# NVlabs/FoundationPose

Hardware: NVIDIA H100
Metric: pose-hypotheses/sec at 640x480 RGB-D, 252 hyp, 5 refine iters (higher is better)
Workload: dtype f16

## Files before the change

foundationpose_b200/csrc/fp_common.cuh:

```cuda
#pragma once
#include <cuda.h>
#include <cuda_fp16.h>
#include <cuda_runtime.h>
#include <stdint.h>
#include <stdio.h>
#include <string.h>

#include <atomic>

namespace fp {

void note_launches(int n);
unsigned long long launch_count();
void set_capturing(bool on);
inline bool device_bit_test(const std::atomic<unsigned long long>& m) {
  int d = 0;
  cudaGetDevice(&d);
  return (m.load(std::memory_order_acquire) >> (d & 63)) & 1ull;
}
inline void device_bit_set(std::atomic<unsigned long long>& m) {
  int d = 0;
  cudaGetDevice(&d);
  m.fetch_or(1ull << (d & 63), std::memory_order_release);
}
int num_sms();

void set_last_error(const char* fmt, ...);
int check_device_ptr(const void* p, const char* what, const char* fn = "fp_pose_errors");
#define FP_CUDA_OK(expr)                                                                   \
  do {                                                                                     \
    cudaError_t _e = (expr);                                                               \
    if (_e != cudaSuccess) {                                                               \
      fp::set_last_error("%s:%d: %s -> %s", __FILE__, __LINE__, #expr, cudaGetErrorString(_e)); \
      return -2;                                                                           \
    }                                                                                      \
  } while (0)
#define FP_REQUIRE(cond, ...)                                                              \
  do {                                                                                     \
    if (!(cond)) {                                                                         \
      fp::set_last_error(__VA_ARGS__);                                                     \
      return -1;                                                                           \
    }                                                                                      \
  } while (0)
#define FP_TRY(expr)     \
  do {                   \
    int _rc = (expr);    \
    if (_rc) return _rc; \
  } while (0)

bool pdl_enabled();
void pdl_skip_next();

template <typename... KArgs, typename... Args>
inline cudaError_t launch_pdl(void (*kernel)(KArgs...), dim3 grid, dim3 block, size_t smem, cudaStream_t stream,
                              int cluster_x, Args... args) {
  cudaLaunchConfig_t cfg;
  memset(&cfg, 0, sizeof(cfg));
  cfg.gridDim = grid;
  cfg.blockDim = block;
  cfg.dynamicSmemBytes = smem;
  cfg.stream = stream;
  cudaLaunchAttribute attr[2];
  int na = 0;
  if (cluster_x > 1) {
    attr[na].id = cudaLaunchAttributeClusterDimension;
    attr[na].val.clusterDim.x = cluster_x;
    attr[na].val.clusterDim.y = 1;
    attr[na].val.clusterDim.z = 1;
    ++na;
  }
  if (pdl_enabled()) {
    attr[na].id = cudaLaunchAttributeProgrammaticStreamSerialization;
    attr[na].val.programmaticStreamSerializationAllowed = 1;
    ++na;
  }
  cfg.attrs = attr;
  cfg.numAttrs = na;
  return cudaLaunchKernelEx(&cfg, kernel, KArgs(args)...);
}

__device__ __forceinline__ void pdl_wait() { asm volatile("griddepcontrol.wait;" ::: "memory"); }
__device__ __forceinline__ void pdl_trigger() { asm volatile("griddepcontrol.launch_dependents;" ::: "memory"); }

__device__ __forceinline__ uint32_t smem_u32(const void* p) {
  return static_cast<uint32_t>(__cvta_generic_to_shared(p));
}

__device__ __forceinline__ void mbar_init(uint64_t* bar, uint32_t count) {
  asm volatile("mbarrier.init.shared::cta.b64 [%0], %1;" ::"r"(smem_u32(bar)), "r"(count));
}
__device__ __forceinline__ void mbar_fence_init() {
  asm volatile("fence.mbarrier_init.release.cluster;" ::: "memory");
}
__device__ __forceinline__ void mbar_expect_tx(uint64_t* bar, uint32_t bytes) {
  asm volatile("mbarrier.arrive.expect_tx.shared::cta.b64 _, [%0], %1;" ::"r"(smem_u32(bar)),
               "r"(bytes)
               : "memory");
}
__device__ __forceinline__ void mbar_arrive(uint64_t* bar) {
  asm volatile("mbarrier.arrive.shared::cta.b64 _, [%0];" ::"r"(smem_u32(bar)) : "memory");
}
__device__ __forceinline__ void mbar_wait(uint64_t* bar, uint32_t parity) {
  asm volatile(
      "{\n\t"
      ".reg .pred P1;\n\t"
      "WAIT_%=:\n\t"
      "mbarrier.try_wait.parity.shared::cta.b64 P1, [%0], %1, %2;\n\t"
      "@P1 bra DONE_%=;\n\t"
      "bra WAIT_%=;\n\t"
      "DONE_%=:\n\t"
      "}" ::"r"(smem_u32(bar)),
      "r"(parity), "r"(0x989680)
      : "memory");
}

__device__ __forceinline__ void tma_load_5d(const CUtensorMap* map, uint64_t* bar, void* dst,
                                            int c0, int c1, int c2, int c3, int c4) {
  asm volatile(
      "cp.async.bulk.tensor.5d.shared::cluster.global.mbarrier::complete_tx::bytes"
      " [%0], [%1, {%3, %4, %5, %6, %7}], [%2];" ::"r"(smem_u32(dst)),
      "l"(reinterpret_cast<uint64_t>(map)), "r"(smem_u32(bar)), "r"(c0), "r"(c1), "r"(c2),
      "r"(c3), "r"(c4)
      : "memory");
}
__device__ __forceinline__ void tma_load_2d(const CUtensorMap* map, uint64_t* bar, void* dst,
                                            int c0, int c1) {
  asm volatile(
      "cp.async.bulk.tensor.2d.shared::cluster.global.mbarrier::complete_tx::bytes"
      " [%0], [%1, {%3, %4}], [%2];" ::"r"(smem_u32(dst)),
      "l"(reinterpret_cast<uint64_t>(map)), "r"(smem_u32(bar)), "r"(c0), "r"(c1)
      : "memory");
}
__device__ __forceinline__ void tma_store_5d(const CUtensorMap* map, const void* src, int c0, int c1, int c2, int c3,
                                             int c4) {
  asm volatile("cp.async.bulk.tensor.5d.global.shared::cta.bulk_group [%0, {%2, %3, %4, %5, %6}], [%1];" ::"l"(
                   reinterpret_cast<uint64_t>(map)),
               "r"(smem_u32(src)), "r"(c0), "r"(c1), "r"(c2), "r"(c3), "r"(c4)
               : "memory");
}
__device__ __forceinline__ void tma_prefetch_desc(const CUtensorMap* map) {
  asm volatile("prefetch.tensormap [%0];" ::"l"(reinterpret_cast<uint64_t>(map)) : "memory");
}

__device__ __forceinline__ uint32_t cluster_nctarank() {
  uint32_t r;
  asm volatile("mov.u32 %0, %%cluster_nctarank;" : "=r"(r));
  return r;
}
__device__ __forceinline__ uint32_t cluster_ctarank() {
  uint32_t r;
  asm volatile("mov.u32 %0, %%cluster_ctarank;" : "=r"(r));
  return r;
}
__device__ __forceinline__ void cluster_sync_all() {
  asm volatile("barrier.cluster.arrive.release.aligned;" ::: "memory");
  asm volatile("barrier.cluster.wait.acquire.aligned;" ::: "memory");
}

template <uint32_t N>
__device__ __forceinline__ void regs_release() {
  asm volatile("setmaxnreg.dec.sync.aligned.u32 %0;" ::"n"(N));
}
template <uint32_t N>
__device__ __forceinline__ void regs_acquire() {
  asm volatile("setmaxnreg.inc.sync.aligned.u32 %0;" ::"n"(N));
}

__device__ __forceinline__ void wgmma_fence() { asm volatile("wgmma.fence.sync.aligned;" ::: "memory"); }
__device__ __forceinline__ void wgmma_commit() { asm volatile("wgmma.commit_group.sync.aligned;" ::: "memory"); }
template <int N>
__device__ __forceinline__ void wgmma_wait() {
  asm volatile("wgmma.wait_group.sync.aligned %0;" ::"n"(N) : "memory");
}
template <int N>
__device__ __forceinline__ void fence_regs(float (&d)[N]) {
#pragma unroll
  for (int i = 0; i < N; ++i) asm volatile("" : "+f"(d[i])::"memory");
}

__device__ __forceinline__ uint64_t gmma_desc_sw128(uint32_t smem_addr, uint32_t sbo = 1024) {
  uint64_t d = 0;
  d |= (uint64_t)((smem_addr & 0x3FFFF) >> 4);
  d |= (uint64_t)1 << 16;
  d |= (uint64_t)(sbo >> 4) << 32;
  d |= (uint64_t)1 << 62;
  return d;
}
__device__ __forceinline__ uint64_t gmma_desc_mn_sw128(uint32_t smem_addr, uint32_t lbo) {
  uint64_t d = 0;
  d |= (uint64_t)((smem_addr & 0x3FFFF) >> 4);
  d |= (uint64_t)((lbo >> 4) & 0x3FFF) << 16;
  d |= (uint64_t)(1024 >> 4) << 32;
  d |= (uint64_t)1 << 62;
  return d;
}
__device__ __forceinline__ uint64_t gmma_desc_linear(uint32_t smem_addr, uint32_t lbo, uint32_t sbo) {
  uint64_t d = 0;
  d |= (uint64_t)((smem_addr & 0x3FFFF) >> 4);
  d |= (uint64_t)(lbo >> 4) << 16;
  d |= (uint64_t)(sbo >> 4) << 32;
  return d;
}

__device__ __forceinline__ void ldsm_x4_trans(uint32_t addr, uint32_t (&r)[4]) {
  asm volatile("ldmatrix.sync.aligned.m8n8.x4.trans.shared.b16 {%0, %1, %2, %3}, [%4];"
               : "=r"(r[0]), "=r"(r[1]), "=r"(r[2]), "=r"(r[3])
               : "r"(addr)
               : "memory");
}
__device__ __forceinline__ void stsm_x4_trans(uint32_t addr, const uint32_t (&r)[4]) {
  asm volatile("stmatrix.sync.aligned.m8n8.x4.trans.shared.b16 [%0], {%1, %2, %3, %4};" ::"r"(addr), "r"(r[0]),
               "r"(r[1]), "r"(r[2]), "r"(r[3])
               : "memory");
}

__device__ __forceinline__ uint32_t pack_half2(float a, float b) {
  __half2 h = __floats2half2_rn(a, b);
  return *reinterpret_cast<uint32_t*>(&h);
}

}
```

foundationpose_b200/csrc/fp_linear.cu:

```cuda
#include <stdlib.h>
#include <string.h>

#include "fp_common.cuh"
#include "fp_gemm.cuh"
#include "fp_wgmma.cuh"

namespace fp {

int encode_map_f16(CUtensorMap* map, const void* base, int rank, const uint64_t* dims, const uint64_t* strides_bytes,
                   const uint32_t* box);

constexpr int kLwsK = 512;
constexpr int kLwsKBlocks = kLwsK / 64;
constexpr int kLwsRows = 64;
constexpr int kLwsCols = 128;
constexpr int kLwsThreads = 384;
constexpr int kLwsBoxBytes = kLwsCols * 64 * 2;
constexpr int kLwsPanelBytes = kLwsKBlocks * kLwsBoxBytes;
constexpr int kLwsStages = kLwsKBlocks;
constexpr int kLwsStageBytes = kLwsRows * 64 * 2;
constexpr int kLwsSlabBytes = kLwsRows * 64 * 2;
constexpr int kLwsSlabs = 4;
constexpr int kLwsSmemBytes =
    kLwsPanelBytes + kLwsStages * kLwsStageBytes + kLwsSlabs * kLwsSlabBytes + 1024  + 256 ;
static_assert(kLwsSmemBytes <= 232448, "the weight-stationary linear kernel exceeds the 227 KB opt-in shared memory");
static_assert((2 * kLwsStages + 4) * 8 <= 256, "the mbarriers must fit their 256 bytes");

constexpr uint32_t kOrderBar = 2;
constexpr uint32_t kWgBar = 4;

struct LinearWsParams {
  int row_tiles;
  int total;
  const float* bias;
  int has_res;
  int relu;
};

__device__ __forceinline__ void named_sync(uint32_t id, uint32_t count) {
  asm volatile("bar.sync %0, %1;" ::"r"(id), "r"(count) : "memory");
}
__device__ __forceinline__ void named_arrive(uint32_t id, uint32_t count) {
  asm volatile("bar.arrive %0, %1;" ::"r"(id), "r"(count) : "memory");
}

__global__ void __launch_bounds__(kLwsThreads, 1)
    linear_ws_kernel(const __grid_constant__ CUtensorMap map_a, const __grid_constant__ CUtensorMap map_w,
                     const __grid_constant__ CUtensorMap map_out, const __grid_constant__ CUtensorMap map_res,
                     const __grid_constant__ LinearWsParams p) {
  extern __shared__ uint8_t smem_raw[];
  uint8_t* smem = smem_raw + ((1024u - (smem_u32(smem_raw) & 1023u)) & 1023u);
  uint8_t* panel = smem;
  uint8_t* ring = panel + kLwsPanelBytes;
  uint8_t* staging = ring + kLwsStages * kLwsStageBytes;
  uint64_t* bars = reinterpret_cast<uint64_t*>(staging + kLwsSlabs * kLwsSlabBytes);
  uint64_t* full = bars;
  uint64_t* empty = bars + kLwsStages;
  uint64_t* panel_full = bars + 2 * kLwsStages;
  uint64_t* panel_empty = panel_full + 1;
  uint64_t* res_full = panel_full + 2;

  const int i0 = (int)((long long)blockIdx.x * p.total / gridDim.x);
  const int n = (int)((long long)(blockIdx.x + 1) * p.total / gridDim.x) - i0;
  const int panel0 = i0 / p.row_tiles;
  const int jb = min(n, (panel0 + 1) * p.row_tiles - i0);
  const bool reload = jb < n;

  if (threadIdx.x == 0) {
    tma_prefetch_desc(&map_a);
    tma_prefetch_desc(&map_w);
    tma_prefetch_desc(&map_out);
    if (p.has_res) tma_prefetch_desc(&map_res);
    for (int s = 0; s < kLwsStages; ++s) {
      mbar_init(&full[s], 1);
      mbar_init(&empty[s], 128);
    }
    mbar_init(panel_full, 1);
    mbar_init(panel_empty, 256);
    mbar_init(&res_full[0], 1);
    mbar_init(&res_full[1], 1);
    mbar_fence_init();
    mbar_expect_tx(panel_full, kLwsPanelBytes);
    for (int kb = 0; kb < kLwsKBlocks; ++kb)
      tma_load_2d(&map_w, panel_full, panel + kb * kLwsBoxBytes, kb * 64, panel0 * kLwsCols);
  }
  __syncthreads();
  pdl_trigger();
  pdl_wait();

  if (threadIdx.x < 128) {
    if (threadIdx.x == 0) {
      for (int j = 0; j < n; ++j) {
        if (j == jb) {
          mbar_wait(panel_empty, 0);
          mbar_expect_tx(panel_full, kLwsPanelBytes);
          for (int kb = 0; kb < kLwsKBlocks; ++kb)
            tma_load_2d(&map_w, panel_full, panel + kb * kLwsBoxBytes, kb * 64, (panel0 + 1) * kLwsCols);
        }
        const int row0 = ((i0 + j) % p.row_tiles) * kLwsRows;
        for (int kb = 0; kb < kLwsKBlocks; ++kb) {
          mbar_wait(&empty[kb], (uint32_t)((j & 1) ^ 1));
          mbar_expect_tx(&full[kb], kLwsStageBytes);
          tma_load_2d(&map_a, &full[kb], ring + kb * kLwsStageBytes, kb * 64, row0);
        }
      }
    }
    return;
  }

  const int ct = threadIdx.x - 128;
  const int w = ct >> 7;
  const int lane = threadIdx.x & 31;
  const int r0 = 16 * ((ct >> 5) & 3) + (lane >> 2);
  const int cq = 2 * (lane & 3);
  const bool leader = (ct & 127) == 0;
  uint8_t* slabs = staging + w * 2 * kLwsSlabBytes;
  if (reload && w >= jb) mbar_arrive(panel_empty);
  float acc[64];
#pragma unroll
  for (int i = 0; i < 64; ++i) acc[i] = 0.f;
  for (int j = w, it = 0; j < n; j += 2, ++it) {
    const int item = i0 + j;
    const int pn = item / p.row_tiles;
    const int row0 = (item - pn * p.row_tiles) * kLwsRows;
    if (j > 0) named_sync(kOrderBar + w, 256);
    mbar_wait(panel_full, j >= jb ? 1u : 0u);
    for (int kb = 0; kb < kLwsKBlocks; ++kb) {
      mbar_wait(&full[kb], (uint32_t)(j & 1));
      const uint64_t da = gmma_desc_sw128(smem_u32(ring + kb * kLwsStageBytes));
      const uint64_t db = gmma_desc_sw128(smem_u32(panel + kb * kLwsBoxBytes));
      wgmma_fence();
#pragma unroll
      for (int k = 0; k < 4; ++k)
        Wgmma<128>::ss(acc, da + (uint64_t)(2 * k), db + (uint64_t)(2 * k), (kb > 0 || k > 0) ? 1u : 0u);
      wgmma_commit();
      if (kb == 0 && leader) {
        asm volatile("cp.async.bulk.wait_group.read 0;" ::: "memory");
        if (p.has_res) {
          mbar_expect_tx(&res_full[w], 2 * kLwsSlabBytes);
          for (int s = 0; s < 2; ++s)
            tma_load_5d(&map_res, &res_full[w], slabs + s * kLwsSlabBytes, pn * kLwsCols + 64 * s, row0, 0, 0, 0);
        }
      }
      if (kb > 0) {
        wgmma_wait<1>();
        mbar_arrive(&empty[kb - 1]);
      }
    }
    if (j + 1 < n) named_arrive(kOrderBar + (w ^ 1), 256);
    wgmma_wait<0>();
    fence_regs(acc);
    mbar_arrive(&empty[kLwsKBlocks - 1]);
    if (reload && j < jb && j + 2 >= jb) mbar_arrive(panel_empty);

    const float* bias = p.bias + pn * kLwsCols;
    if (p.has_res) mbar_wait(&res_full[w], (uint32_t)(it & 1));
    else named_sync(kWgBar + w, 128);
#pragma unroll
    for (int b = 0; b < 2; ++b) {
      uint8_t* slab = slabs + b * kLwsSlabBytes;
#pragma unroll
      for (int jh = 0; jh < 8; jh += 4) {
        float2 bb[4];
        __half2 rv[4][2];
#pragma unroll
        for (int jl = 0; jl < 4; ++jl) {
          bb[jl] = __ldg(reinterpret_cast<const float2*>(bias + 64 * b + 8 * (jh + jl) + cq));
          if (p.has_res) {
#pragma unroll
            for (int h = 0; h < 2; ++h) {
              const int row = r0 + 8 * h;
              rv[jl][h] = *reinterpret_cast<const __half2*>(slab + row * 128 + (((uint32_t)(jh + jl) ^ (uint32_t)(row & 7)) << 4) + cq * 2);
            }
          }
        }
#pragma unroll
        for (int jl = 0; jl < 4; ++jl) {
          const int jc = 8 * b + jh + jl;
#pragma unroll
          for (int h = 0; h < 2; ++h) {
            const int row = r0 + 8 * h;
            uint32_t* cell = reinterpret_cast<uint32_t*>(slab + row * 128 + (((uint32_t)(jh + jl) ^ (uint32_t)(row & 7)) << 4) + cq * 2);
            float a0 = acc[4 * jc + 2 * h] + bb[jl].x, a1 = acc[4 * jc + 2 * h + 1] + bb[jl].y;
            if (p.has_res) {
              const float2 r = __half22float2(rv[jl][h]);
              a0 += r.x;
              a1 += r.y;
            }
            if (p.relu) {
              a0 = fmaxf(a0, 0.f);
              a1 = fmaxf(a1, 0.f);
            }
            *cell = pack_half2(a0, a1);
          }
        }
      }
    }
    asm volatile("fence.proxy.async.shared::cta;" ::: "memory");
    named_sync(kWgBar + w, 128);
    if (leader) {
      for (int s = 0; s < 2; ++s)
        tma_store_5d(&map_out, slabs + s * kLwsSlabBytes, pn * kLwsCols + 64 * s, row0, 0, 0, 0);
      asm volatile("cp.async.bulk.commit_group;" ::: "memory");
    }
  }
  if (leader) asm volatile("cp.async.bulk.wait_group 0;" ::: "memory");
}

static bool linear_ws_enabled() {
  const char* e = getenv("FPOSE_LINEAR_WS");
  return !(e && e[0] == '0');
}

constexpr int kLinearWsMinItemsPerCta = 8;

bool linear_ws_takes(const GemmLayer& L) {
  if (L.kind != LK_LINEAR || L.Cin != kLwsK || L.Cout % kLwsCols != 0 || L.out_split != 0 || L.post_add ||
      !linear_ws_enabled())
    return false;
  const int sms = num_sms();
  const int panels = L.Cout / kLwsCols;
  const long long items = (long long)panels * ((L.Win + kLwsRows - 1) / kLwsRows);
  return sms > 0 && panels <= sms && items >= (long long)kLinearWsMinItemsPerCta * sms;
}

int linear_ws_launch(const GemmLayer& L, cudaStream_t stream) {
  const uint64_t E = 2;
  const int M = L.Win;
  LinearWsParams p;
  memset(&p, 0, sizeof(p));
  p.row_tiles = (M + kLwsRows - 1) / kLwsRows;
  p.total = (L.Cout / kLwsCols) * p.row_tiles;
  p.bias = L.bias;
  p.has_res = L.res != nullptr;
  p.relu = L.relu;
  CUtensorMap ma, mw, mo, mr;
  {
    const uint64_t d[2] = {(uint64_t)kLwsK, (uint64_t)M}, s[1] = {(uint64_t)kLwsK * E};
    const uint32_t b[2] = {64, kLwsRows};
    if (int rc = encode_map_f16(&ma, L.in, 2, d, s, b)) return rc;
  }
  {
    const uint64_t d[2] = {(uint64_t)kLwsK, (uint64_t)L.Cout}, s[1] = {(uint64_t)kLwsK * E};
    const uint32_t b[2] = {64, kLwsCols};
    if (int rc = encode_map_f16(&mw, L.w, 2, d, s, b)) return rc;
  }
  auto rows_map = [&](CUtensorMap* m, const void* base, int ld) {
    const uint64_t row = (uint64_t)ld * E;
    const uint64_t d[5] = {(uint64_t)ld, (uint64_t)M, 1, 1, 1}, s[4] = {row, row * M, row * M, row * M};
    const uint32_t b[5] = {64, kLwsRows, 1, 1, 1};
    return encode_map_f16(m, base, 5, d, s, b);
  };
  if (int rc = rows_map(&mo, L.out, L.out_ld)) return rc;
  mr = mo;
  if (L.res) {
    if (int rc = rows_map(&mr, L.res, L.res_ld)) return rc;
  }

  static std::atomic<unsigned long long> attr_mask{0};
  if (!device_bit_test(attr_mask)) {
    FP_CUDA_OK(cudaFuncSetAttribute(linear_ws_kernel, cudaFuncAttributeMaxDynamicSharedMemorySize, kLwsSmemBytes));
    device_bit_set(attr_mask);
  }
  const int sms = num_sms();
  FP_REQUIRE(sms > 0, "no CUDA device");
  const int grid = p.total < sms ? p.total : sms;
  prof_mark_begin(0, 2.0 * (double)M * L.Cout * kLwsK, stream);
  FP_CUDA_OK(launch_pdl(linear_ws_kernel, dim3(grid), dim3(kLwsThreads), kLwsSmemBytes, stream, 1, ma, mw, mo, mr, p));
  prof_mark_end(stream);
  note_launches(1);
  FP_CUDA_OK(cudaGetLastError());
  return 0;
}

}
```

foundationpose_b200/csrc/fp_stem.cu:

```cuda
#include <stdlib.h>
#include <string.h>

#include "fp_common.cuh"
#include "fp_gemm.cuh"
#include "fp_wgmma.cuh"

namespace fp {

int encode_map_f16(CUtensorMap* map, const void* base, int rank, const uint64_t* dims, const uint64_t* strides_bytes,
                   const uint32_t* box);
int encode_map_f16_linear(CUtensorMap* map, const void* base, int rank, const uint64_t* dims,
                          const uint64_t* strides_bytes, const uint32_t* box);
int num_sms();

namespace {

constexpr int kThreadsStem = 384;
constexpr int kTileH = 16, kTileW = 8;
constexpr int kPatchRows = 2 * (kTileH - 1) + 7;
constexpr int kPatchPairs = kTileW + 3;
constexpr int kParStride = kPatchPairs * 16;
constexpr int kRowStride = 2 * kParStride;
constexpr int kPatchBytes = kPatchRows * kRowStride;
constexpr int kPatchSlot = 13 * 1024;
constexpr int kStagesStem = 6;
constexpr int kWTileBytes = 2 * 64 * 16;
constexpr int kWBytes = 28 * kWTileBytes;
constexpr int kHalfSlab = 64 * 64 * 2;
constexpr int kStemSmem = kWBytes + kStagesStem * kPatchSlot + 4 * kHalfSlab + 1024 + 256;

struct StemParams {
  int tiles_w, tiles_h, n_img, total_tiles;
  const float* bias;
  int relu;
};

__device__ __forceinline__ void bulk_load_1d(void* dst, const void* src, uint32_t bytes, uint64_t* bar) {
  asm volatile("cp.async.bulk.shared::cluster.global.mbarrier::complete_tx::bytes [%0], [%1], %2, [%3];" ::"r"(
                   smem_u32(dst)),
               "l"(src), "r"(bytes), "r"(smem_u32(bar))
               : "memory");
}

__global__ void __launch_bounds__(kThreadsStem, 1)
    stem_conv_kernel(const __grid_constant__ CUtensorMap map_in, const __grid_constant__ CUtensorMap map_out,
                     const __half* __restrict__ wpack, const StemParams p) {
  constexpr int S = kStagesStem;
  extern __shared__ uint8_t smem_raw[];
  uint8_t* smem = reinterpret_cast<uint8_t*>((reinterpret_cast<uintptr_t>(smem_raw) + 1023) & ~uintptr_t(1023));
  uint8_t* wsm = smem;
  uint8_t* ring = smem + kWBytes;
  uint8_t* staging = ring + S * kPatchSlot;
  uint64_t* bars = reinterpret_cast<uint64_t*>(staging + 4 * kHalfSlab);
  uint64_t* full = bars;
  uint64_t* empty = bars + S;
  uint64_t* w_full = bars + 2 * S;

  if (threadIdx.x == 0) {
    tma_prefetch_desc(&map_in);
    tma_prefetch_desc(&map_out);
    for (int s = 0; s < S; ++s) {
      mbar_init(&full[s], 1);
      mbar_init(&empty[s], 256);
    }
    mbar_init(w_full, 1);
    mbar_fence_init();
  }
  __syncthreads();
  const int tiles_per_img = p.tiles_w * p.tiles_h;
  pdl_trigger();

  if (threadIdx.x < 128) {
    if (threadIdx.x == 0) {
      mbar_expect_tx(w_full, kWBytes);
      bulk_load_1d(wsm, wpack, kWBytes, w_full);
      pdl_wait();
      int stage = 0, phase = 0;
      for (int t = blockIdx.x; t < p.total_tiles; t += gridDim.x) {
        const int n = t / tiles_per_img, rem = t - n * tiles_per_img;
        const int th = rem / p.tiles_w, tw = rem - th * p.tiles_w;
        mbar_wait(&empty[stage], phase ^ 1);
        mbar_expect_tx(&full[stage], kPatchBytes);
        tma_load_5d(&map_in, &full[stage], ring + stage * kPatchSlot, tw * kTileW * 8, 0, th * 2 * kTileH, n, 0);
        if (++stage == S) {
          stage = 0;
          phase ^= 1;
        }
      }
    }
    return;
  }

  const int ct = threadIdx.x - 128;
  const int cw = ct >> 7;
  const int lane = threadIdx.x & 31;
  const int r0 = 16 * ((ct >> 5) & 3) + (lane >> 2);
  const int cq = 2 * (lane & 3);
  const bool leader = ((ct & 127) == 0);
  const uint32_t w_addr = smem_u32(wsm);
  float2 bias[8];
#pragma unroll
  for (int j = 0; j < 8; ++j) bias[j] = __ldg(reinterpret_cast<const float2*>(p.bias + 8 * j + cq));
  float acc[32];
#pragma unroll
  for (int i = 0; i < 32; ++i) acc[i] = 0.f;
  mbar_wait(w_full, 0);
  pdl_wait();
  int stage = 0, phase = 0, use = 0;
  for (int t = blockIdx.x; t < p.total_tiles; t += gridDim.x, ++use) {
    const int n = t / tiles_per_img, rem = t - n * tiles_per_img;
    const int th = rem / p.tiles_w, tw = rem - th * p.tiles_w;
    mbar_wait(&full[stage], phase);
    const uint32_t patch = smem_u32(ring + stage * kPatchSlot) + (uint32_t)(cw * 8 * 2 * kRowStride);
    wgmma_fence();
#pragma unroll
    for (int r = 0; r < 7; ++r) {
#pragma unroll
      for (int s = 0; s < 4; ++s) {
        const uint64_t da = gmma_desc_linear(patch + r * kRowStride + s * 16, kParStride, 2 * kRowStride);
        const uint64_t db = gmma_desc_linear(w_addr + (r * 4 + s) * kWTileBytes, 1024, 128);
        Wgmma<64>::ss(acc, da, db, (r | s) ? 1u : 0u);
      }
    }
    wgmma_commit();
    wgmma_wait<0>();
    fence_regs(acc);
    mbar_arrive(&empty[stage]);
    if (++stage == S) {
      stage = 0;
      phase ^= 1;
    }

    uint8_t* slab = staging + (cw * 2 + (use & 1)) * kHalfSlab;
    if (leader) asm volatile("cp.async.bulk.wait_group.read 1;" ::: "memory");
    asm volatile("bar.sync %0, 128;" ::"r"(1 + cw) : "memory");
#pragma unroll
    for (int j = 0; j < 8; ++j) {
#pragma unroll
      for (int h = 0; h < 2; ++h) {
        const int row = r0 + 8 * h;
        float a0 = acc[4 * j + 2 * h] + bias[j].x, a1 = acc[4 * j + 2 * h + 1] + bias[j].y;
        if (p.relu) {
          a0 = fmaxf(a0, 0.f);
          a1 = fmaxf(a1, 0.f);
        }
        *reinterpret_cast<uint32_t*>(slab + row * 128 + (((uint32_t)j ^ (uint32_t)(row & 7)) << 4) + cq * 2) =
            pack_half2(a0, a1);
      }
    }
    asm volatile("fence.proxy.async.shared::cta;" ::: "memory");
    asm volatile("bar.sync %0, 128;" ::"r"(1 + cw) : "memory");
    if (leader) {
      tma_store_5d(&map_out, slab, 0, tw * kTileW, th * kTileH + 8 * cw, n, 0);
      asm volatile("cp.async.bulk.commit_group;" ::: "memory");
    }
  }
  if (leader) asm volatile("cp.async.bulk.wait_group 0;" ::: "memory");
}

}

int stem_conv_launch(const GemmLayer& L, cudaStream_t stream) {
  FP_REQUIRE(L.Cin == 8 && L.Cout == 64, "CONV7_S2: the stem kernel is 8 (6 + 2 zero) -> 64 channels");
  FP_REQUIRE(L.Hin % (2 * kTileH) == 0 && L.Win % (2 * kTileW) == 0, "CONV7_S2: unsupported size %dx%d", L.Hin, L.Win);
  FP_REQUIRE(!L.res && !L.post_add && L.out_split == 0, "CONV7_S2: residual / post-add / split are not supported");
  FP_REQUIRE(L.out_ld % 8 == 0 && L.out_ld >= 64, "CONV7_S2: bad out_ld %d", L.out_ld);
  FP_REQUIRE((reinterpret_cast<uintptr_t>(L.w) & 15) == 0, "CONV7_S2: weights must be 16-byte aligned");
  if (L.n_img == 0) return 0;
  const int Ho = L.Hin / 2, Wo = L.Win / 2;
  const uint64_t E = 2;
  const uint64_t rows = L.Hin + 6, pairs = (L.Win + 8) / 2;
  CUtensorMap mi, mo;
  {
    uint64_t d[5] = {8 * pairs, 2, rows, (uint64_t)L.n_img, 1};
    uint64_t s[4] = {pairs * 8 * E, 2 * pairs * 8 * E, rows * 2 * pairs * 8 * E, rows * 2 * pairs * 8 * E * L.n_img};
    uint32_t b[5] = {8 * (uint32_t)kPatchPairs, 2, (uint32_t)kPatchRows, 1, 1};
    int rc = encode_map_f16_linear(&mi, L.in, 5, d, s, b);
    if (rc) return rc;
  }
  {
    uint64_t d[5] = {(uint64_t)L.out_ld, (uint64_t)Wo, (uint64_t)Ho, (uint64_t)L.n_img, 1};
    uint64_t s[4] = {(uint64_t)L.out_ld * E, (uint64_t)L.out_ld * E * Wo, (uint64_t)L.out_ld * E * Wo * Ho,
                     (uint64_t)L.out_ld * E * Wo * Ho * L.n_img};
    uint32_t b[5] = {64, (uint32_t)kTileW, (uint32_t)kTileH / 2, 1, 1};
    int rc = encode_map_f16(&mo, L.out, 5, d, s, b);
    if (rc) return rc;
  }
  StemParams p;
  p.tiles_w = Wo / kTileW;
  p.tiles_h = Ho / kTileH;
  p.n_img = L.n_img;
  p.total_tiles = p.tiles_w * p.tiles_h * L.n_img;
  p.bias = L.bias;
  p.relu = L.relu;
  static std::atomic<unsigned long long> attr_mask{0};
  if (!device_bit_test(attr_mask)) {
    FP_CUDA_OK(cudaFuncSetAttribute(stem_conv_kernel, cudaFuncAttributeMaxDynamicSharedMemorySize, kStemSmem));
    device_bit_set(attr_mask);
  }
  const int sms = num_sms();
  FP_REQUIRE(sms > 0, "no CUDA device");
  const int grid = p.total_tiles < sms ? p.total_tiles : sms;
  prof_mark_begin(0, 2.0 * (double)L.n_img * Ho * Wo * 64.0 * (7.0 * 7.0 * 6.0), stream);
  FP_CUDA_OK(launch_pdl(stem_conv_kernel, dim3(grid), dim3(kThreadsStem), kStemSmem, stream, 1, mi, mo,
                        reinterpret_cast<const __half*>(L.w), p));
  prof_mark_end(stream);
  note_launches(1);
  FP_CUDA_OK(cudaGetLastError());
  return 0;
}

}
```

Before: 3988.

## Swap stem wgmma operands so each warpgroup owns whole tiles with ping-pong ordering

The stem conv now treats weights as the A operand and the patch pixels as B, with an N=128 wgmma. Each of the two consumer warpgroups therefore computes a full tile on its own, where before it computed half a tile. The warpgroups alternate tiles and use named barriers to order their wgmma issue, so one group's epilogue overlaps the other's MMA. The epilogue writes results with stmatrix transposed stores and issues two TMA stores per tile. This doubles the accumulator registers per thread to 64 floats and doubles the staging shared memory, which may raise register pressure.

```diff
diff --git a/foundationpose_b200/csrc/fp_common.cuh b/foundationpose_b200/csrc/fp_common.cuh
--- a/foundationpose_b200/csrc/fp_common.cuh
+++ b/foundationpose_b200/csrc/fp_common.cuh
@@ -157,6 +157,13 @@
   asm volatile("barrier.cluster.wait.acquire.aligned;" ::: "memory");
 }
 
+__device__ __forceinline__ void named_sync(uint32_t id, uint32_t count) {
+  asm volatile("bar.sync %0, %1;" ::"r"(id), "r"(count) : "memory");
+}
+__device__ __forceinline__ void named_arrive(uint32_t id, uint32_t count) {
+  asm volatile("bar.arrive %0, %1;" ::"r"(id), "r"(count) : "memory");
+}
+
 template <uint32_t N>
 __device__ __forceinline__ void regs_release() {
   asm volatile("setmaxnreg.dec.sync.aligned.u32 %0;" ::"n"(N));
diff --git a/foundationpose_b200/csrc/fp_linear.cu b/foundationpose_b200/csrc/fp_linear.cu
--- a/foundationpose_b200/csrc/fp_linear.cu
+++ b/foundationpose_b200/csrc/fp_linear.cu
@@ -37,13 +37,6 @@
   int relu;
 };
 
-__device__ __forceinline__ void named_sync(uint32_t id, uint32_t count) {
-  asm volatile("bar.sync %0, %1;" ::"r"(id), "r"(count) : "memory");
-}
-__device__ __forceinline__ void named_arrive(uint32_t id, uint32_t count) {
-  asm volatile("bar.arrive %0, %1;" ::"r"(id), "r"(count) : "memory");
-}
-
 __global__ void __launch_bounds__(kLwsThreads, 1)
     linear_ws_kernel(const __grid_constant__ CUtensorMap map_a, const __grid_constant__ CUtensorMap map_w,
                      const __grid_constant__ CUtensorMap map_out, const __grid_constant__ CUtensorMap map_res,
diff --git a/foundationpose_b200/csrc/fp_stem.cu b/foundationpose_b200/csrc/fp_stem.cu
--- a/foundationpose_b200/csrc/fp_stem.cu
+++ b/foundationpose_b200/csrc/fp_stem.cu
@@ -26,8 +26,14 @@
 constexpr int kStagesStem = 6;
 constexpr int kWTileBytes = 2 * 64 * 16;
 constexpr int kWBytes = 28 * kWTileBytes;
-constexpr int kHalfSlab = 64 * 64 * 2;
-constexpr int kStemSmem = kWBytes + kStagesStem * kPatchSlot + 4 * kHalfSlab + 1024 + 256;
+constexpr int kSlab = kTileH * kTileW * 64 * 2;
+constexpr int kHalfSlab = kSlab / 2;
+constexpr int kStemSmem = kWBytes + kStagesStem * kPatchSlot + 4 * kSlab + 1024 + 256;
+static_assert(kStemSmem <= 232448, "the stem kernel exceeds the 227 KB opt-in shared memory");
+static_assert((2 * kStagesStem + 1) * 8 <= 256, "the mbarriers must fit their 256 bytes");
+
+constexpr uint32_t kOrderBar = 2;
+constexpr uint32_t kWgBar = 4;
 
 struct StemParams {
   int tiles_w, tiles_h, n_img, total_tiles;
@@ -51,7 +57,7 @@
   uint8_t* wsm = smem;
   uint8_t* ring = smem + kWBytes;
   uint8_t* staging = ring + S * kPatchSlot;
-  uint64_t* bars = reinterpret_cast<uint64_t*>(staging + 4 * kHalfSlab);
+  uint64_t* bars = reinterpret_cast<uint64_t*>(staging + 4 * kSlab);
   uint64_t* full = bars;
   uint64_t* empty = bars + S;
   uint64_t* w_full = bars + 2 * S;
@@ -61,13 +67,14 @@
     tma_prefetch_desc(&map_out);
     for (int s = 0; s < S; ++s) {
       mbar_init(&full[s], 1);
-      mbar_init(&empty[s], 256);
+      mbar_init(&empty[s], 128);
     }
     mbar_init(w_full, 1);
     mbar_fence_init();
   }
   __syncthreads();
   const int tiles_per_img = p.tiles_w * p.tiles_h;
+  const int nt = (p.total_tiles - (int)blockIdx.x + (int)gridDim.x - 1) / (int)gridDim.x;
   pdl_trigger();
 
   if (threadIdx.x < 128) {
@@ -76,7 +83,8 @@
       bulk_load_1d(wsm, wpack, kWBytes, w_full);
       pdl_wait();
       int stage = 0, phase = 0;
-      for (int t = blockIdx.x; t < p.total_tiles; t += gridDim.x) {
+      for (int j = 0; j < nt; ++j) {
+        const int t = blockIdx.x + j * gridDim.x;
         const int n = t / tiles_per_img, rem = t - n * tiles_per_img;
         const int th = rem / p.tiles_w, tw = rem - th * p.tiles_w;
         mbar_wait(&empty[stage], phase ^ 1);
@@ -92,66 +100,68 @@
   }
 
   const int ct = threadIdx.x - 128;
-  const int cw = ct >> 7;
+  const int w = ct >> 7;
+  const int wq = (ct >> 5) & 3;
   const int lane = threadIdx.x & 31;
-  const int r0 = 16 * ((ct >> 5) & 3) + (lane >> 2);
-  const int cq = 2 * (lane & 3);
-  const bool leader = ((ct & 127) == 0);
+  const bool leader = (ct & 127) == 0;
   const uint32_t w_addr = smem_u32(wsm);
-  float2 bias[8];
-#pragma unroll
-  for (int j = 0; j < 8; ++j) bias[j] = __ldg(reinterpret_cast<const float2*>(p.bias + 8 * j + cq));
-  float acc[32];
-#pragma unroll
-  for (int i = 0; i < 32; ++i) acc[i] = 0.f;
+  uint8_t* slabs = staging + w * 2 * kSlab;
+  const float bc[2] = {__ldg(p.bias + 16 * wq + (lane >> 2)), __ldg(p.bias + 16 * wq + (lane >> 2) + 8)};
+  const int mi = lane >> 3, mr = lane & 7;
+  const uint32_t lane_off = (uint32_t)(8 * (mi >> 1) + mr) * 128u + ((uint32_t)((2 * wq + (mi & 1)) ^ mr) << 4);
+  float acc[64];
+#pragma unroll
+  for (int i = 0; i < 64; ++i) acc[i] = 0.f;
   mbar_wait(w_full, 0);
   pdl_wait();
-  int stage = 0, phase = 0, use = 0;
-  for (int t = blockIdx.x; t < p.total_tiles; t += gridDim.x, ++use) {
+  for (int j = w, it = 0; j < nt; j += 2, ++it) {
+    const int t = blockIdx.x + j * gridDim.x;
     const int n = t / tiles_per_img, rem = t - n * tiles_per_img;
     const int th = rem / p.tiles_w, tw = rem - th * p.tiles_w;
-    mbar_wait(&full[stage], phase);
-    const uint32_t patch = smem_u32(ring + stage * kPatchSlot) + (uint32_t)(cw * 8 * 2 * kRowStride);
+    const int stage = j % S;
+    if (j > 0) named_sync(kOrderBar + w, 256);
+    mbar_wait(&full[stage], (uint32_t)((j / S) & 1));
+    const uint32_t patch = smem_u32(ring + stage * kPatchSlot);
     wgmma_fence();
 #pragma unroll
     for (int r = 0; r < 7; ++r) {
 #pragma unroll
       for (int s = 0; s < 4; ++s) {
-        const uint64_t da = gmma_desc_linear(patch + r * kRowStride + s * 16, kParStride, 2 * kRowStride);
-        const uint64_t db = gmma_desc_linear(w_addr + (r * 4 + s) * kWTileBytes, 1024, 128);
-        Wgmma<64>::ss(acc, da, db, (r | s) ? 1u : 0u);
+        const uint64_t da = gmma_desc_linear(w_addr + (r * 4 + s) * kWTileBytes, 1024, 128);
+        const uint64_t db = gmma_desc_linear(patch + r * kRowStride + s * 16, kParStride, 2 * kRowStride);
+        Wgmma<128>::ss(acc, da, db, (r | s) ? 1u : 0u);
       }
     }
     wgmma_commit();
+    if (j + 1 < nt) named_arrive(kOrderBar + (w ^ 1), 256);
+    uint8_t* slab = slabs + (it & 1) * kSlab;
+    if (leader) asm volatile("cp.async.bulk.wait_group.read 1;" ::: "memory");
     wgmma_wait<0>();
     fence_regs(acc);
     mbar_arrive(&empty[stage]);
-    if (++stage == S) {
-      stage = 0;
-      phase ^= 1;
-    }
-
-    uint8_t* slab = staging + (cw * 2 + (use & 1)) * kHalfSlab;
-    if (leader) asm volatile("cp.async.bulk.wait_group.read 1;" ::: "memory");
-    asm volatile("bar.sync %0, 128;" ::"r"(1 + cw) : "memory");
-#pragma unroll
-    for (int j = 0; j < 8; ++j) {
-#pragma unroll
-      for (int h = 0; h < 2; ++h) {
-        const int row = r0 + 8 * h;
-        float a0 = acc[4 * j + 2 * h] + bias[j].x, a1 = acc[4 * j + 2 * h + 1] + bias[j].y;
+    named_sync(kWgBar + w, 128);
+
+    const uint32_t slab_addr = smem_u32(slab) + lane_off;
+#pragma unroll
+    for (int g = 0; g < 8; ++g) {
+      uint32_t o[4];
+#pragma unroll
+      for (int i = 0; i < 4; ++i) {
+        const int jj = 2 * g + (i >> 1), h = i & 1;
+        float a0 = acc[4 * jj + 2 * h] + bc[h], a1 = acc[4 * jj + 2 * h + 1] + bc[h];
         if (p.relu) {
           a0 = fmaxf(a0, 0.f);
           a1 = fmaxf(a1, 0.f);
         }
-        *reinterpret_cast<uint32_t*>(slab + row * 128 + (((uint32_t)j ^ (uint32_t)(row & 7)) << 4) + cq * 2) =
-            pack_half2(a0, a1);
+        o[i] = pack_half2(a0, a1);
       }
+      stsm_x4_trans(slab_addr + g * 2048u, o);
     }
     asm volatile("fence.proxy.async.shared::cta;" ::: "memory");
-    asm volatile("bar.sync %0, 128;" ::"r"(1 + cw) : "memory");
+    named_sync(kWgBar + w, 128);
     if (leader) {
-      tma_store_5d(&map_out, slab, 0, tw * kTileW, th * kTileH + 8 * cw, n, 0);
+      tma_store_5d(&map_out, slab, 0, tw * kTileW, th * kTileH, n, 0);
+      tma_store_5d(&map_out, slab + kHalfSlab, 0, tw * kTileW, th * kTileH + kTileH / 2, n, 0);
       asm volatile("cp.async.bulk.commit_group;" ::: "memory");
     }
   }
```

New measurement: 4032, median of 6. 1.1% higher.
